# soedinglab/MMseqs2

Hardware: AMD Instinct MI355X
Metric: sw_gcells_per_s (higher is better)
Workload: dtype int16

## Files before the change

### mmseqs2_amd/csrc/pf_kernels.hip

```cpp
#include <type_traits>

#include "mmgpu_internal.h"
#include "pf_device.h"

namespace mmgpu {

namespace {

__device__ __forceinline__ PfCand *cand_slot(const PfDedupArgs &A, uint64_t bucket, uint32_t k) {
    return k < (uint32_t)PF_CAND0 ? A.cand_small + bucket * PF_CAND0 + k : A.cand + (A.cand_base[bucket] - A.cand_origin) + k;
}

struct __attribute__((packed, aligned(4))) U32Pair {
    uint32_t a, b;
};
struct __attribute__((packed, aligned(4))) U32Quad {
    uint32_t a, b, c, d;
};


constexpr uint32_t PF_COFS_KMERS = 12, PF_COFS_DWORDS = 4;

__global__ __launch_bounds__(256) void pf_cofs_kernel(const uint32_t *offsets, uint64_t table, uint32_t *cofs) {
    const uint64_t blk = (uint64_t)blockIdx.x * 256u + threadIdx.x;
// ... 447 lines not shown
            if (chunk_end > cur) cur = chunk_end;
            L += 64;
            r = rn;
            if (L >= Lend) break;
        }
    }
    __syncthreads();

    const int nbits = pf_bin_shift(B);
    constexpr int ROUNDS = PF_T / (64 * SPW);
    uint64_t ent[ROUNDS];
    uint32_t rk[ROUNDS];
    uint16_t *mycnt = cnt + (uint32_t)wave * B;
#pragma unroll
    for (int r = 0; r < ROUNDS; r++) {
        const uint32_t slot = (uint32_t)wave * (PF_T / SPW) + (uint32_t)r * 64u + (uint32_t)lane;
        const bool valid = slot < tile_n;
        ent[r] = valid ? stage[slot] : 0ull;
        const uint32_t bin = (uint32_t)ent[r] & (B - 1);
        const uint64_t m = match_lanes(bin, nbits, valid);
        const uint32_t rank = (uint32_t)__popcll(m & lanes_below(lane));
        uint32_t c = 0;
        if (valid) c = mycnt[bin];
        rk[r] = c + rank;
        if (valid && rank == 0) mycnt[bin] = (uint16_t)(c + (uint32_t)__popcll(m));
    }
    __syncthreads();

    {
        const uint32_t bpt = B >= 256 ? B / 256 : 1;
        const uint32_t b0 = threadIdx.x * bpt;
        uint32_t s = 0;
        if (b0 < B)
            for (uint32_t b = b0; b < b0 + bpt; b++)
                for (int w = 0; w < SPW; w++) s += cnt[(uint32_t)w * B + b];
        const uint32_t incl = wave_incl_scan(s);
        if (lane == 63) wsum[wave] = incl;
        __syncthreads();
        uint32_t run = incl - s;
        for (int w = 0; w < wave; w++) run += wsum[w];
        if (b0 < B) {
            uint16_t *bo = A.bin_off + (size_t)t * (B + 1);
            for (uint32_t b = b0; b < b0 + bpt; b++) {
                bo[b] = (uint16_t)run;
                uint32_t tot = 0;
                for (int w = 0; w < SPW; w++) {
                    const uint32_t c = cnt[(uint32_t)w * B + b];
                    cnt[(uint32_t)w * B + b] = (uint16_t)(run + tot);
                    tot += c;
                }
                if (tot) atomicAdd(&A.bucket_count[(size_t)q * B + b], tot);
                run += tot;
            }
            if (b0 + bpt == B) bo[B] = (uint16_t)run;
        }
    }
    __syncthreads();

    uint32_t *stage_w = reinterpret_cast<uint32_t *>(stage);
    uint8_t *stage_h = reinterpret_cast<uint8_t *>(stage) + (size_t)PF_T * 4;
#pragma unroll
    for (int r = 0; r < ROUNDS; r++) {
        const uint32_t slot = (uint32_t)wave * (PF_T / SPW) + (uint32_t)r * 64u + (uint32_t)lane;
        if (slot < tile_n) {
            const uint32_t id = (uint32_t)ent[r];
            const uint32_t bin = id & (B - 1);
            const uint32_t diag = (uint32_t)(ent[r] >> 32) & 0xFFFFu;
            const uint32_t at = mycnt[bin] + rk[r];
            stage_w[at] = (id >> nbits) | ((diag & 0xFFu) << 12) | ((uint32_t)(ent[r] >> 48) << 20);
            stage_h[at] = (uint8_t)(diag >> 8);
        }
    }
    __syncthreads();
    uint32_t *dst = A.split + (size_t)t * PF_T;
    uint32_t *dst_h = reinterpret_cast<uint32_t *>(A.split_hi + (size_t)t * PF_T);
    const uint32_t *src_h = reinterpret_cast<const uint32_t *>(stage_h);
    for (uint32_t s = threadIdx.x; s < tile_n; s += (uint32_t)SPW * 64u) dst[s] = stage_w[s];
    for (uint32_t s = threadIdx.x; s < (tile_n + 3u) / 4u; s += (uint32_t)SPW * 64u) dst_h[s] = src_h[s];
}

struct Seg {
    int a, b, P, M;
};
__device__ __forceinline__ Seg seg_combine(const Seg &l, const Seg &r) {
    Seg o;
    o.b = l.b + r.b;
    o.a = max(r.a, l.a + r.b);
    o.P = max(l.P, l.b + r.P);
    o.M = max(max(l.M, r.M), l.a + r.P);
    return o;
}
template <int NW>
__device__ __forceinline__ void load_cells(const uint8_t *p, uint32_t (&w)[NW]) {
    static_assert(NW == 4 || NW == 6, "16 or 24 bytes");
    const uintptr_t u = reinterpret_cast<uintptr_t>(p);
    const uint32_t *a = reinterpret_cast<const uint32_t *>(u & ~(uintptr_t)3);
    const uint32_t sh = (uint32_t)(u & 3u);
    const U32Quad d = *reinterpret_cast<const U32Quad *>(a);
    w[0] = __builtin_amdgcn_alignbyte(d.b, d.a, sh);
    w[1] = __builtin_amdgcn_alignbyte(d.c, d.b, sh);
    w[2] = __builtin_amdgcn_alignbyte(d.d, d.c, sh);
    if constexpr (NW == 4) {
        w[3] = __builtin_amdgcn_alignbyte(a[4], d.d, sh);
    } else {
        typedef uint32_t u32x3 __attribute__((ext_vector_type(3)));
        const u32x3 e = *reinterpret_cast<const u32x3 *>(a + 4);
        w[3] = __builtin_amdgcn_alignbyte(e.x, d.d, sh);
        w[4] = __builtin_amdgcn_alignbyte(e.y, e.x, sh);
        w[5] = __builtin_amdgcn_alignbyte(e.z, e.y, sh);
    }
}
template <int NW>
__device__ __forceinline__ Seg seg_cells_n(const uint32_t (&tw)[NW], const uint32_t (&qw)[NW], const uint32_t (&cw)[NW], int nn,
                                           const int8_t *smat) {
    Seg g;
    g.a = 0; g.b = 0; g.P = -(1 << 28); g.M = 0;
#pragma unroll
    for (int k = 0; k < 4 * NW; k++) {
        const uint32_t t5 = (tw[k >> 2] >> ((k & 3) * 8)) & 31u;
        const uint32_t q5 = (qw[k >> 2] >> ((k & 3) * 8)) & 31u;
        const int cb = (int)(int8_t)((cw[k >> 2] >> ((k & 3) * 8)) & 0xFFu);
        int x = (int)(int8_t)(smat[(q5 << 5) | t5] + cb);
        x = k < nn ? x : 0;
        g.b += x;
        g.a = max(0, g.a + x);
        g.P = max(g.P, g.b);
        g.M = max(g.M, g.a);
    }
    return g;
}
template <int NW>
__device__ __forceinline__ Seg seg_cells_rows_n(const uint32_t (&tw)[NW], const int8_t *rows, int nn) {
    Seg g;
    g.a = 0; g.b = 0; g.P = -(1 << 28); g.M = 0;
#pragma unroll
    for (int k = 0; k < 4 * NW; k++) {
        if (k < nn) {
            const int tb_ = (int)((tw[k >> 2] >> ((k & 3) * 8)) & 0xFFu);
            const int x = (int)rows[k * PF_PROW + (tb_ & (PF_PROW - 1))];
            g.b += x;
            g.a = max(0, g.a + x);
            g.P = max(g.P, g.b);
            g.M = max(g.M, g.a);
        }
    }
    return g;
}
__device__ __forceinline__ Seg seg_tree16(Seg g, int gl) {
#pragma unroll
    for (int d = 1; d < 16; d <<= 1) {
        Seg r;
        r.a = __shfl_down(g.a, d);
        r.b = __shfl_down(g.b, d);
        r.P = __shfl_down(g.P, d);
        r.M = __shfl_down(g.M, d);
        if ((gl & (2 * d - 1)) == 0) g = seg_combine(g, r);
    }
    return g;
}

template <bool SLOTS = true>
__device__ __forceinline__ uint64_t score_chunk(const PfDedupArgs &A, const int8_t *smat, uint64_t bucket, uint32_t q, uint32_t cb0,
                                                uint32_t nin, uint32_t ncand, PfCand c, int bshift, uint32_t *score_out = nullptr) {
    const int lane = lane_id();
    const int grp = lane >> 4, gl = lane & 15;
    const uint32_t qp0 = A.q_off[q];
    const int qlen = (int)(A.q_off[q + 1] - qp0);
    const uint8_t *qr = A.q_res + qp0;
    const uint8_t *qc = reinterpret_cast<const uint8_t *>(A.q_corr) + qp0;
    const bool has = (uint32_t)lane < nin;
    const int8_t *prows = (A.q_isprof && A.q_isprof[q]) ? A.q_rows + (size_t)qp0 * PF_PROW : nullptr;
    int my_len = 0, my_qs = 0;
    unsigned long long my_addr = 0;
    uint64_t cells = 0;
    if (has && !(A.q_nseg && A.q_nseg[q]))
        c.diag = (uint16_t)((c.diag & 0xFFu) | ((uint32_t)A.split_hi[(size_t)A.q_tile_base[q] * PF_T + c.score] << 8));
    if (has) {
        const int d = (int)(short)c.diag;
        const int tlen = (int)A.t_len[c.id];
        const uint8_t *t = A.t_res + (size_t)A.t_off4[c.id] * 4;
        const int mind = d < 0 ? -d : d;
        int ts = 0;
        if (d >= 0 && mind < qlen) {
            my_len = min(tlen, qlen - mind);
            my_qs = mind;
        } else if (d < 0 && mind < tlen) {
            my_len = min(tlen - mind, qlen);
            ts = mind;
        }
        my_addr = (unsigned long long)reinterpret_cast<uintptr_t>(t + ts);
        cells = (uint64_t)my_len;
        if (tlen >= 32768 && A.q_flags) atomicOr(&A.q_flags[q], 1u);
    }
    int my_score = 0;
    constexpr int UN = 2;
    auto trip = [&](auto nw_tag, const uint32_t k0) {
        constexpr int NW = decltype(nw_tag)::value;
        constexpr int CPL = 4 * NW, PASS = 16 * CPL;
        uint32_t tw[UN][NW], qw[UN][NW], cw[UN][NW];
        int len_u[UN], qs_u[UN];
        unsigned long long addr_u[UN];
#pragma unroll
        for (int u = 0; u < UN; u++) {
            const int src = (int)k0 + u * 4 + grp;
            len_u[u] = __shfl(my_len, src);
            qs_u[u] = __shfl(my_qs, src);
            addr_u[u] = __shfl(my_addr, src);
            if ((uint32_t)src >= nin) len_u[u] = 0;
#pragma unroll
            for (int z = 0; z < NW; z++) { tw[u][z] = 0; qw[u][z] = 0; cw[u][z] = 0; }
            if (gl * CPL < len_u[u]) {
                load_cells<NW>(reinterpret_cast<const uint8_t *>((uintptr_t)addr_u[u]) + gl * CPL, tw[u]);
                if (!prows) {
                    load_cells<NW>(qr + qs_u[u] + gl * CPL, qw[u]);
                    load_cells<NW>(qc + qs_u[u] + gl * CPL, cw[u]);
                }
            }
        }
#pragma unroll
        for (int u = 0; u < UN; u++) {
            const int len = len_u[u];
            Seg g;
            g.a = 0; g.b = 0; g.P = -(1 << 28); g.M = 0;
            if (gl * CPL < len) {
                if (prows) g = seg_cells_rows_n<NW>(tw[u], prows + (size_t)(qs_u[u] + gl * CPL) * PF_PROW, min(CPL, len - gl * CPL));
                else g = seg_cells_n<NW>(tw[u], qw[u], cw[u], min(CPL, len - gl * CPL), smat);
            }
            g = seg_tree16(g, gl);
            int sc = 0, best = 0;
            if (gl == 0 && len > 0) {
                best = max(g.M, g.P);
                sc = max(g.a, g.b);
            }
            int maxlen = len;
            maxlen = max(maxlen, __shfl_xor(maxlen, 16));
            maxlen = max(maxlen, __shfl_xor(maxlen, 32));
            for (int p0 = PASS; p0 < maxlen; p0 += PASS) {
                const int o = p0 + gl * CPL;
                Seg h;
                h.a = 0; h.b = 0; h.P = -(1 << 28); h.M = 0;
                if (o < len) {
                    uint32_t t2[NW], q2[NW], c2[NW];
                    load_cells<NW>(reinterpret_cast<const uint8_t *>((uintptr_t)addr_u[u]) + o, t2);
                    if (prows) h = seg_cells_rows_n<NW>(t2, prows + (size_t)(qs_u[u] + o) * PF_PROW, min(CPL, len - o));
                    else {
                        load_cells<NW>(qr + qs_u[u] + o, q2);
                        load_cells<NW>(qc + qs_u[u] + o, c2);
                        h = seg_cells_n<NW>(t2, q2, c2, min(CPL, len - o), smat);
                    }
                }
                h = seg_tree16(h, gl);
                if (gl == 0 && p0 < len) {
                    best = max(best, max(h.M, sc + h.P));
                    sc = max(h.a, sc + h.b);
                }
            }
            const int r0 = __shfl(best, 0), r1 = __shfl(best, 16), r2 = __shfl(best, 32), r3 = __shfl(best, 48);
            const int rel = lane - ((int)k0 + u * 4);
            if (rel >= 0 && rel < 4) my_score = rel == 0 ? r0 : (rel == 1 ? r1 : (rel == 2 ? r2 : r3));
        }
    };
    for (uint32_t k0 = 0; k0 < nin; k0 += 4 * UN) {
        const bool mine = (uint32_t)lane >= k0 && (uint32_t)lane < k0 + 4u * UN && has;
        if (ballot(mine && my_len > 256)) trip(std::integral_constant<int, 6>{}, k0);
        else trip(std::integral_constant<int, 4>{}, k0);
    }
    c.score = (uint32_t)my_score;
    if (score_out) *score_out = c.score;
    if constexpr (!SLOTS) return cells;
    if (has) {
        PfCand *slot = cand_slot(A, bucket, cb0 + (uint32_t)lane);
        slot->score = c.score;
        slot->diag = c.diag;
    }
    if (ncand <= 64 && !A.nucl) {
        const uint32_t cnt = min(255u, c.score);
        const uint64_t same = match_lanes(c.id >> bshift, 12, has);
        bool win = has;
        uint64_t m = same & ~(1ull << lane);
        while (ballot(m != 0)) {
            const int o = m ? __ffsll((long long)m) - 1 : lane;
            const uint32_t oc = __shfl(cnt, o);
            if (m) {
                if (oc > cnt || (oc == cnt && o < lane)) win = false;
                m &= m - 1;
            }
        }
        win = win && cnt >= A.min_diag_score;
        const uint64_t wb = ballot(win);
        if (wb) {
            PfCand *surv = A.surv + (A.cand_base[(uint64_t)q * A.bins] - A.cand_origin);
            uint32_t base = 0;
            if (lane == 0) base = atomicAdd(&A.surv_count[q], (uint32_t)__popcll(wb));
            base = __shfl(base, 0);
            if (win) surv[base + (uint32_t)__popcll(wb & lanes_below(lane))] = c;
        }
    }
    return cells;
}

constexpr int REPLAY_WAVES_PER_EU = 4;
constexpr int REPLAY_PD = 4;


struct ReplayLds {
    uint32_t prev[4][PF_IDS_PER_BIN / 4];
    uint32_t last[4][PF_IDS_PER_BIN / 4];
    uint32_t emit[4][PF_IDS_PER_BIN / 32];
    uint32_t cand[4][3][64];
    uint8_t mark[4][64];
    int8_t smat[32 * 32];
};

__device__ __forceinline__ uint32_t lds_byte_exchange(uint32_t *word, uint32_t shift, uint32_t byte) {
    uint32_t old;
    const uint32_t addr = (uint32_t)(uintptr_t)word;
    asm volatile("ds_mskor_rtn_b32 %0, %1, %2, %3\n\ts_waitcnt lgkmcnt(0)" : "=v"(old) : "v"(addr), "v"(0xFFu << shift), "v"(byte << shift) : "memory");
    return old;
}

template <bool SEGS>
__device__ __forceinline__ void replay_bucket_impl(const PfDedupArgs &A, ReplayLds &M, uint64_t bucket) {
    const int lane = lane_id(), wave = (int)(threadIdx.x >> 6);
    const uint32_t B = A.bins;
    const uint32_t q = (uint32_t)(bucket / B), bin = (uint32_t)(bucket % B);
    const uint32_t ntiles = A.q_ntiles[q];
    if (ntiles == 0) {
        if (lane == 0) A.cand_count[bucket] = 0;
        return;
    }
    const uint32_t tb = A.q_tile_base[q];
    uint32_t *P = M.prev[wave];
    uint32_t *L = M.last[wave];
    uint32_t *E = M.emit[wave];
    uint8_t *mark = M.mark[wave];
    const int bshift = pf_bin_shift(B);
    auto clear_state = [&]() {
        uint4 *P4 = reinterpret_cast<uint4 *>(P);
        for (int k = lane; k < PF_IDS_PER_BIN / 16; k += 64) P4[k] = make_uint4(0u, 0u, 0u, 0u);
        for (int k = lane; k < PF_IDS_PER_BIN / 32; k += 64) E[k] = 0;
    };
    clear_state();

    uint32_t ncand = 0;
    const uint64_t below = lanes_below(lane);
    PfCand *const cand_small = A.cand_small + bucket * PF_CAND0;
    PfCand *const cand_big = A.cand + (A.cand_base[bucket] - A.cand_origin);
    const uint8_t *const split_hi_q = A.split_hi + (size_t)tb * PF_T;
    const uint32_t *const split_q = A.split + (size_t)tb * PF_T;
    const uint32_t nseg = SEGS ? A.q_nseg[q] : 0u;
// ... 24 lines not shown
            const uint32_t d_m = (uint32_t)__shfl((int)seg_delta, m);
            tile_out = t0 + (uint32_t)m;
            at_out = (uint32_t)(x + d_m);
            e_out = split_q[x < total ? (size_t)tile_out * PF_T + at_out : (size_t)0];
        };
        auto one_round = [&](const uint32_t x0, uint32_t &e_slot, uint32_t &tile_slot, uint32_t &at_slot) {
            const uint32_t e = e_slot;
            const uint32_t tile_cur = tile_slot;
            const uint32_t where = tile_cur * (uint32_t)PF_T + at_slot;
            const bool act = x0 + (uint32_t)lane < total;
            request(x0 + 64u * REPLAY_PD, e_slot, tile_slot, at_slot);
            const uint32_t key = e & 0xFFFu;
            const uint32_t d8 = (e >> 12) & 0xFFu;
            const uint32_t arr = tile_cur * (uint32_t)PF_T + (e >> 20);
            const uint32_t sh = (key & 3u) * 8u;
            uint64_t todo = SEGS ? ballot(act) : 1ull;
            while (todo) {
                const bool now = SEGS ? (act && ((todo >> lane) & 1ull) && arr < next_boundary) : act;
                if (!SEGS || ballot(now)) {
                    bool flag = false;
                    if (now) flag = ((lds_byte_exchange(&P[key >> 2], sh, d8) >> sh) & 0xFFu) == d8;
                    if (ballot(flag)) {
                        bool keep = false;
                        if (flag) {
                            const uint32_t bit = 1u << (key & 31u);
                            const bool emitted_before = (atomicOr(&E[key >> 5], bit) & bit) != 0u;
                            const uint32_t last_byte = (lds_byte_exchange(&L[key >> 2], sh, d8) >> sh) & 0xFFu;
                            keep = !emitted_before || last_byte != d8;
                        }
                        const uint64_t kb = ballot(keep);
                        if (keep) {
                            PfCand c;
                            c.id = (key << bshift) | bin;
                            c.arr = arr;
                            c.score = SEGS ? 0u : where;
                            c.diag = (uint16_t)(SEGS ? (d8 | ((uint32_t)split_hi_q[where] << 8)) : d8);
                            c.pad = (uint16_t)cur_seg;
                            const uint32_t ck = ncand + (uint32_t)__popcll(kb & below);
                            *(ck < (uint32_t)PF_CAND0 ? cand_small + ck : cand_big + ck) = c;
                            if (!SEGS && ck < 64) {
                                M.cand[wave][0][ck] = key | (d8 << 12);
                                M.cand[wave][1][ck] = arr;
                                M.cand[wave][2][ck] = where;
                            }
                        }
                        ncand += (uint32_t)__popcll(kb);
                    }
                }
                if (!SEGS) break;
                todo &= ~ballot(now);
                if (todo) {
                    clear_state();
                    cur_seg++;
                    next_boundary = cur_seg + 1 <= nseg ? segs[cur_seg + 1] : 0xFFFFFFFFu;
                }
            }
        };
        static_assert(REPLAY_PD == 4, "four named slots below");
        uint32_t e0, e1, e2, e3, tile0, tile1, tile2, tile3, at0, at1, at2, at3;
        request(0u, e0, tile0, at0);
        request(64u, e1, tile1, at1);
        request(128u, e2, tile2, at2);
        request(192u, e3, tile3, at3);
        for (uint32_t xg = 0; xg < total; xg += 64u * REPLAY_PD) {
            one_round(xg, e0, tile0, at0);
            one_round(xg + 64u, e1, tile1, at1);
            one_round(xg + 128u, e2, tile2, at2);
            one_round(xg + 192u, e3, tile3, at3);
        }
    }
    if (lane == 0) {
        A.cand_count[bucket] = ncand;
        if (!SEGS && ncand > 64 && A.big_list) A.big_list[atomicAdd(A.big_count, 1u)] = (uint32_t)(bucket - (uint64_t)A.q_first * B);
    }
    if (!SEGS && ncand > 0 && ncand <= 64) {
        PfCand c = pf_cand_zero();
        if ((uint32_t)lane < ncand) {
            const uint32_t kd = M.cand[wave][0][lane];
            c.id = ((kd & 0xFFFu) << bshift) | bin;
            c.arr = M.cand[wave][1][lane];
            c.diag = (uint16_t)(kd >> 12);
            c.score = M.cand[wave][2][lane];
        }
        uint64_t cells = score_chunk(A, M.smat, bucket, q, 0, ncand, ncand, c, bshift);
        if (A.cell_counter) wave_sum_to((unsigned long long *)&A.cell_counter[q], cells);
    }
}

__global__ __launch_bounds__(256) __attribute__((amdgpu_waves_per_eu(REPLAY_WAVES_PER_EU))) void pf_replay_kernel(PfDedupArgs A) {
    __shared__ ReplayLds M;
    pf_load_smat32<256>(M.smat, A.mat, A.alphabet);
    __syncthreads();
    uint64_t bucket;
    if (!pf_wave_bucket(A, 4u, &bucket)) return;
    if (A.q_nseg && A.q_nseg[(uint32_t)(bucket / A.bins)]) replay_bucket_impl<true>(A, M, bucket);
    else replay_bucket_impl<false>(A, M, bucket);
}

__device__ __forceinline__ void ungapped_bucket(const PfDedupArgs &A, const int8_t *smat, uint64_t bucket) {
    const int lane = lane_id();
    const uint32_t B = A.bins;
    const uint32_t ncand = A.cand_count[bucket];
    const uint32_t q = (uint32_t)(bucket / B);
    if (ncand <= 64 || (A.q_nseg && A.q_nseg[q])) return;
    const int bshift = pf_bin_shift(B);
    uint64_t cells = 0;
    for (uint32_t cb0 = 0; cb0 < ncand; cb0 += 64) {
        const uint32_t nin = min(64u, ncand - cb0);
        PfCand c = pf_cand_zero();
        if ((uint32_t)lane < nin) c = *cand_slot(A, bucket, cb0 + (uint32_t)lane);
        cells += score_chunk(A, smat, bucket, q, cb0, nin, ncand, c, bshift);
    }
    if (A.cell_counter) wave_sum_to((unsigned long long *)&A.cell_counter[q], cells);
}

__global__ __launch_bounds__(256) void pf_ungapped_kernel(PfDedupArgs A) {
    __shared__ int8_t smat[32 * 32];
    const int wave = (int)(threadIdx.x >> 6);
    pf_load_smat32<256>(smat, A.mat, A.alphabet);
    __syncthreads();
    const uint32_t B = A.bins;
    if (A.big_list) {
        const uint32_t n = *A.big_count;
        for (uint32_t i = blockIdx.x * 4u + (uint32_t)wave; i < n; i += gridDim.x * 4u) ungapped_bucket(A, smat, (uint64_t)A.q_first * B + A.big_list[i]);
        return;
    }
    const uint64_t bucket = (uint64_t)A.q_first * B + (uint64_t)blockIdx.x * 4u + (uint32_t)wave;
    if (bucket >= (uint64_t)(A.q_first + A.n_queries) * B) return;
    ungapped_bucket(A, smat, bucket);
}

__global__ __launch_bounds__(256) void pf_count_kernel(PfDedupArgs A) {
    __shared__ uint16_t s_state[4][PF_IDS_PER_BIN];
    __shared__ uint32_t s_emit[4][PF_IDS_PER_BIN / 32];
    const int lane = lane_id(), wave = (int)(threadIdx.x >> 6);
    const uint32_t B = A.bins;
    uint64_t bucket;
    if (!pf_wave_bucket(A, 4u, &bucket)) return;
    const uint32_t q = (uint32_t)(bucket / B), bin = (uint32_t)(bucket % B);
    const uint32_t ntiles = A.q_ntiles[q];
    if (lane == 0) A.cand_count[bucket] = 0;
    if (ntiles == 0) return;
    const uint32_t tb = A.q_tile_base[q];
    uint16_t *S = s_state[wave];
    uint32_t *E = s_emit[wave];
    const int bshift = pf_bin_shift(B);
    for (int k = lane; k < PF_IDS_PER_BIN; k += 64) S[k] = 0;
    for (int k = lane; k < PF_IDS_PER_BIN / 32; k += 64) E[k] = 0;
    uint32_t ncand = 0;
    const uint64_t below = lanes_below(lane);
    for (uint32_t t0 = 0; t0 < ntiles; t0 += 64) {
        const uint32_t tl = t0 + (uint32_t)lane;
        uint32_t o0 = 0, n = 0;
        if (tl < ntiles) {
            const uint16_t *bo = A.bin_off + (size_t)(tb + tl) * (B + 1) + bin;
            o0 = bo[0];
            n = (uint32_t)bo[1] - o0;
        }
        const uint32_t incl = wave_incl_scan(n);
        const uint32_t total = __shfl(incl, 63);
        const uint32_t excl = incl - n;
        for (uint32_t x0 = 0; x0 < total; x0 += 64) {
            const uint32_t x = x0 + (uint32_t)lane;
            const bool now = x < total;
            const int m = seg_find(excl, now ? x : 0u);
            const uint32_t ex_m = __shfl(excl, m), o_m = __shfl(o0, m);
            const uint32_t tile = t0 + (uint32_t)m;
            uint32_t e = 0;
            const size_t where = (size_t)(tb + tile) * PF_T + o_m + (x - ex_m);
            if (now) e = A.split[where];
            const uint32_t key = e & 0xFFFu;
            const uint32_t id = (key << bshift) | bin;
            const uint32_t d8 = (e >> 12) & 0xFFu;
            const uint32_t arr = tile * (uint32_t)PF_T + (e >> 20);
            const uint64_t same = match_lanes(key, 12, now);
            uint32_t st = 0, em = 0;
            if (now) {
                st = S[key];
                em = (E[key >> 5] >> (key & 31u)) & 1u;
            }
            const uint64_t pm = same & below;
            const int pl = pm ? highest_lane(pm) : lane;
            const uint32_t d_pl = __shfl(d8, pl);
            const uint32_t prevd = pm ? d_pl : (st & 0xFFu);
            const bool flag = now && d8 == prevd;
            const uint64_t fl = ballot(flag);
            const uint64_t fm = same & fl;
            if (now && (same & ~below & ~(1ull << lane)) == 0) {
                const uint32_t cnt = min(255u, (st >> 8) + (uint32_t)__popcll(fm));
                S[key] = (uint16_t)(d8 | (cnt << 8));
            }
            const bool keep = flag && (fm & below) == 0 && em == 0u;
            if (keep) atomicOr(&E[key >> 5], 1u << (key & 31u));
            const uint64_t kb = ballot(keep);
            if (keep) {
                PfCand c;
                c.id = id;
                c.arr = arr;
                c.score = 0;
                c.diag = (uint16_t)(d8 | ((uint32_t)A.split_hi[where] << 8));
                c.pad = 0;
                *cand_slot(A, bucket, ncand + (uint32_t)__popcll(kb & below)) = c;
            }
            ncand += (uint32_t)__popcll(kb);
        }
    }
    if (ncand == 0) return;
    __threadfence();
    if (lane == 0 && A.q_ncand) {
        const uint32_t before = atomicAdd(&A.q_ncand[q], ncand);
        if (before + ncand >= A.sort_cap && A.q_flags) atomicOr(&A.q_flags[q], 2u);
    }
// ... 38 lines not shown
            c = *cand_slot(A, bucket, ci);
            const uint32_t cnt = min(255u, c.score);
            win = S[c.id >> bshift] == keepmax_key(cnt, ci) && cnt >= A.min_diag_score;
        }
        wave_append(&A.surv_count[q], surv, win, c);
    }
}

__global__ __launch_bounds__(256) void pf_keepmax_kernel(PfDedupArgs A) {
    __shared__ uint32_t s_tab[4][PF_IDS_PER_BIN];
    const int wave = (int)(threadIdx.x >> 6);
    if (A.nucl) return;
    uint64_t bucket;
    if (!pf_wave_bucket(A, 4u, &bucket)) return;
    keepmax_bucket(A, s_tab[wave], bucket);
}

__global__ __launch_bounds__(1024) void pf_keepmax_list_kernel(PfDedupArgs A) {
    __shared__ uint32_t S[PF_IDS_PER_BIN];
    const uint32_t B = A.bins;
    const int bshift = pf_bin_shift(B);
    const uint32_t n = *A.big_count;
    for (uint32_t i = blockIdx.x; i < n; i += gridDim.x) {
        const uint64_t bucket = (uint64_t)A.q_first * B + A.big_list[i];
        const uint32_t ncand = A.cand_count[bucket];
        const uint32_t q = (uint32_t)(bucket / B);
        for (uint32_t k = threadIdx.x; k < (uint32_t)PF_IDS_PER_BIN; k += 1024) S[k] = 0;
        __syncthreads();
        for (uint32_t ci = threadIdx.x; ci < ncand; ci += 1024) {
            const PfCand *cp = cand_slot(A, bucket, ci);
            atomicMax(&S[cp->id >> bshift], keepmax_key(min(255u, cp->score), ci));
        }
        __syncthreads();
        PfCand *surv = A.surv + (A.cand_base[(uint64_t)q * B] - A.cand_origin);
        for (uint32_t c0 = 0; c0 < ncand; c0 += 1024) {
            const uint32_t ci = c0 + threadIdx.x;
            bool win = false;
            PfCand c = pf_cand_zero();
            if (ci < ncand) {
                c = *cand_slot(A, bucket, ci);
                const uint32_t cnt = min(255u, c.score);
                win = S[c.id >> bshift] == keepmax_key(cnt, ci) && cnt >= A.min_diag_score;
            }
            wave_append(&A.surv_count[q], surv, win, c);
        }
        __syncthreads();
    }
}

constexpr int PF_LONG_POOL = 4096;
constexpr uint32_t PF_LONG_NONE = 0xFFFFu;

__device__ int wave_diag_score(const int8_t *smat, const uint8_t *qr, const uint8_t *qc, const int8_t *prows, int qlen, const uint8_t *t,
                               int tlen, int diag) {
    const int lane = lane_id();
    const int mind = diag < 0 ? -diag : diag;
    int len, qs, ts;
    if (diag >= 0 && mind < qlen) {
        len = min(tlen, qlen - mind);
        qs = mind;
        ts = 0;
    } else if (diag < 0 && mind < tlen) {
        len = min(tlen - mind, qlen);
        qs = 0;
        ts = mind;
    } else {
        return 0;
    }
    int sc = 0, best = 0;
    for (int p0 = 0; p0 < len; p0 += 1024) {
        const int o = p0 + lane * 16;
        Seg h;
        h.a = 0; h.b = 0; h.P = -(1 << 28); h.M = 0;
        if (o < len) {
            uint32_t tw[4], qw[4], cw[4];
            load_cells<4>(t + ts + o, tw);
            if (prows) h = seg_cells_rows_n<4>(tw, prows + (size_t)(qs + o) * PF_PROW, min(16, len - o));
            else {
                load_cells<4>(qr + qs + o, qw);
                load_cells<4>(qc + qs + o, cw);
                h = seg_cells_n<4>(tw, qw, cw, min(16, len - o), smat);
            }
        }
        h = seg_tree16(h, lane & 15);
        Seg g[4];
#pragma unroll
        for (int k = 0; k < 4; k++) {
            g[k].a = __shfl(h.a, 16 * k);
            g[k].b = __shfl(h.b, 16 * k);
            g[k].P = __shfl(h.P, 16 * k);
            g[k].M = __shfl(h.M, 16 * k);
        }
        const Seg all = seg_combine(seg_combine(g[0], g[1]), seg_combine(g[2], g[3]));
        best = max(best, max(all.M, sc + all.P));
        sc = max(all.a, sc + all.b);
    }
    return best;
}

__device__ int wave_long_score(const int8_t *smat, const uint8_t *qr, const uint8_t *qc, const int8_t *prows, int qlen, const uint8_t *t,
                               int tlen, uint32_t diag16) {
    int total = 0;
    for (uint32_t d = 1; d <= 1u + (uint32_t)tlen / 32768u; d++)
        total = max(total, wave_diag_score(smat, qr, qc, prows, qlen, t, tlen, (int)(0u - d * 65536u + diag16)));
    for (uint32_t d = 0; d <= (uint32_t)qlen / 65536u; d++)
        total = max(total, wave_diag_score(smat, qr, qc, prows, qlen, t, tlen, (int)(d * 65536u + diag16)));
    return total;
}

__global__ __launch_bounds__(256) void pf_longq_kernel(PfDedupArgs A) {
    __shared__ int8_t smat[32 * 32];
    const int lane = lane_id();
    pf_load_smat32<256>(smat, A.mat, A.alphabet);
    __syncthreads();
    const uint32_t B = A.bins;
    uint64_t bucket;
    if (!pf_wave_bucket(A, 4u, &bucket)) return;
    const uint32_t q = (uint32_t)(bucket / B);
    const uint32_t qp0 = A.q_off[q];
    const int qlen = (int)(A.q_off[q + 1] - qp0);
    if (qlen < 32768) return;
    if (lane == 0 && bucket == (uint64_t)q * B) atomicOr(&A.q_flags[q], 1u);
    if (A.nucl || (A.q_nseg && A.q_nseg[q])) return;
    const uint8_t *qr = A.q_res + qp0;
    const uint8_t *qc = reinterpret_cast<const uint8_t *>(A.q_corr) + qp0;
    const int8_t *prows = (A.q_isprof && A.q_isprof[q]) ? A.q_rows + (size_t)qp0 * PF_PROW : nullptr;
    const uint32_t ncand = A.cand_count[bucket];
    for (uint32_t ci = 0; ci < ncand; ci++) {
        PfCand *slot = cand_slot(A, bucket, ci);
        const uint32_t id = slot->id;
        const int own = wave_long_score(smat, qr, qc, prows, qlen, A.t_res + (size_t)A.t_off4[id] * 4, (int)A.t_len[id], slot->diag);
        if (lane == 0) slot->score = (uint32_t)own;
    }
}

__global__ __launch_bounds__(256) void pf_long_kernel(PfDedupArgs A) {
    __shared__ uint32_t s_tab[PF_IDS_PER_BIN];
    __shared__ uint32_t s_dbits[65536 / 32];
    __shared__ uint64_t s_key[PF_LONG_POOL];
    __shared__ uint32_t s_ci[PF_LONG_POOL];
    __shared__ uint16_t s_bucket[PF_LONG_POOL];
    __shared__ uint16_t s_job[PF_LONG_POOL];
    __shared__ int8_t smat[32 * 32];
    __shared__ uint32_t sh_npool, sh_nlong;
    const uint32_t q = A.q_first + blockIdx.x;
    if (!(A.q_flags[q] & 1u)) return;
    if (A.nucl || (A.q_nseg && A.q_nseg[q])) return;
    const int lane = lane_id(), wave = (int)(threadIdx.x >> 6);
    const uint32_t B = A.bins;
    const int bshift = pf_bin_shift(B);
    pf_load_smat32<256>(smat, A.mat, A.alphabet);
    for (int k = (int)threadIdx.x; k < 65536 / 32; k += 256) s_dbits[k] = 0;
    if (threadIdx.x == 0) {
        sh_npool = 0;
        sh_nlong = 0;
    }
    __syncthreads();
    const uint32_t qp0 = A.q_off[q];
    const int qlen = (int)(A.q_off[q + 1] - qp0);
    if (qlen < 32768) {
    for (uint32_t bk = (uint32_t)wave; bk < B; bk += 4) {
        const uint64_t bucket = (uint64_t)q * B + bk;
        const uint32_t ncand = A.cand_count[bucket];
        for (uint32_t ci = (uint32_t)lane; ci < ncand; ci += 64) {
            const PfCand *cp = cand_slot(A, bucket, ci);
            if (A.t_len[cp->id] >= 32768u) atomicOr(&s_dbits[cp->diag >> 5], 1u << (cp->diag & 31u));
        }
    }
    __syncthreads();
    const uint32_t refmask = A.ref_bins - 1;
    for (uint32_t bk = (uint32_t)wave; bk < B; bk += 4) {
        const uint64_t bucket = (uint64_t)q * B + bk;
        const uint32_t ncand = A.cand_count[bucket];
        for (uint32_t ci = (uint32_t)lane; ci < ncand; ci += 64) {
            const PfCand *cp = cand_slot(A, bucket, ci);
            const uint32_t d = cp->diag;
// ... 265 lines not shown
        for (uint32_t r0 = 0; r0 < n; r0 += 64) {
            const bool act = r0 + (uint32_t)lane < n;
            const uint32_t idx = act ? n - 1u - (r0 + (uint32_t)lane) : 0u;
            PfOvfElem e;
            e.id = 0; e.score = 0; e.ord = 0; e.diag = 0; e.pad0 = 0; e.pad1 = 0;
            if (act) e = O[idx];
            const uint32_t d8 = e.diag & 0xFFu, key = e.id >> bshift;
            const uint64_t same = match_lanes(key, 12, act);
            const uint64_t pm = same & below;
            const int pl = pm ? highest_lane(pm) : lane;
            const uint32_t d_pl = __shfl(d8, pl);
            uint32_t prev = 0;
            if (act) prev = pm ? d_pl : tab[key];
            const bool keep = act && (e.score != 0 || prev != d8);
            if (act && (same & ~below & ~(1ull << lane)) == 0) tab[key] = d8;
            const uint64_t kb = ballot(keep);
            if (keep) {
                e.ord = -e.ord;
                S[m + (uint32_t)__popcll(kb & below)] = e;
            }
            m += (uint32_t)__popcll(kb);
        }
        n = m;
        cur = S;
    } else if (do_merge && final_step) {
        for (uint32_t r0 = 0; r0 < n; r0 += 64) {
            const bool act = r0 + (uint32_t)lane < n;
            const uint32_t idx = act ? n - 1u - (r0 + (uint32_t)lane) : 0u;
            uint32_t id = 0, d8 = 0;
            if (act) { id = O[idx].id; d8 = O[idx].diag & 0xFFu; }
            const uint32_t key = id >> bshift;
            const uint64_t same = match_lanes(key, 12, act);
            if (act && (same & ~below & ~(1ull << lane)) == 0) tab[key] = (d8 + 1u) & 0xFFu;
        }
        uint32_t m = 0;
        for (uint32_t r0 = 0; r0 < n; r0 += 64) {
            const uint32_t idx = r0 + (uint32_t)lane;
            const bool act = idx < n;
            PfOvfElem e;
            e.id = 0; e.score = 0; e.ord = 0; e.diag = 0; e.pad0 = 0; e.pad1 = 0;
            if (act) e = O[idx];
            const uint32_t d8 = e.diag & 0xFFu, key = e.id >> bshift;
            const uint64_t same = match_lanes(key, 12, act);
            const uint64_t pm = same & below;
            const int pl = pm ? highest_lane(pm) : lane;
            const uint32_t d_pl = __shfl(d8, pl);
            uint32_t prev = 0;
            if (act) prev = pm ? d_pl : tab[key];
            const bool keep = act && prev != d8;
            if (act && (same & ~below & ~(1ull << lane)) == 0) tab[key] = d8;
            const uint64_t kb = ballot(keep);
            if (keep) S[m + (uint32_t)__popcll(kb & below)] = e;
            m += (uint32_t)__popcll(kb);
        }
        n = m;
        cur = S;
    }
    __threadfence();
    const bool do_score = final_step || (step > 1 && prev_total != 0);
    if (!do_score) {
        if (lane == 0) {
            A.o_count[(size_t)qi * B + bin] = n;
            if (n) atomicAdd(&totals[step], n);
        }
        return;
    }
    for (uint32_t r0 = 0; r0 < n; r0 += 64) {
        const uint32_t idx = r0 + (uint32_t)lane;
        const bool need = idx < n && cur[idx].score == 0;
        const uint64_t nb = ballot(need);
        if (!nb) continue;
        const uint32_t cnt = (uint32_t)__popcll(nb), mine = (uint32_t)__popcll(nb & below);
        if (need) tab[mine] = (uint32_t)lane;
        __builtin_amdgcn_wave_barrier();
        const int src = (uint32_t)lane < cnt ? (int)tab[lane] : 0;
        const uint32_t my_id = idx < n ? cur[idx].id : 0u, my_diag = idx < n ? (uint32_t)cur[idx].diag : 0u;
        PfCand c;
        c.id = (uint32_t)__shfl((int)my_id, src);
        c.arr = 0;
        c.score = 0;
        c.diag = (uint16_t)__shfl((int)my_diag, src);
        c.pad = 0;
        uint32_t sc = 0;
        (void)score_chunk<false>(D, smat, bucket, q, 0, cnt, 65u, c, bshift, &sc);
        tab[64 + lane] = sc;
        __builtin_amdgcn_wave_barrier();
        if (need) cur[idx].score = tab[64 + mine];
    }
    __threadfence();
    for (int k = lane; k < PF_IDS_PER_BIN; k += 64) tab[k] = 0;
    for (uint32_t r0 = 0; r0 < n; r0 += 64) {
        const uint32_t idx = r0 + (uint32_t)lane;
        if (idx < n) {
            const uint32_t cnt = min(255u, cur[idx].score);
            atomicMax(&tab[cur[idx].id >> bshift], keepmax_key(cnt, idx));
        }
    }
    PfOvfElem *dst = cur == O ? S : O;
    uint32_t m = 0;
    PfCand *surv = D.surv + (D.cand_base[(uint64_t)q * B] - D.cand_origin);
    for (uint32_t r0 = 0; r0 < n; r0 += 64) {
        const uint32_t idx = r0 + (uint32_t)lane;
        bool keep = false;
        PfOvfElem e;
        e.id = 0; e.score = 0; e.ord = 0; e.diag = 0; e.pad0 = 0; e.pad1 = 0;
        if (idx < n) {
            e = cur[idx];
            const uint32_t cnt = min(255u, e.score);
            const uint32_t first = 0xFFFFFFu - (tab[e.id >> bshift] & 0xFFFFFFu);
            keep = idx == first || (cnt == 0 && idx > first);
            if (final_step) keep = keep && cnt >= D.min_diag_score;
        }
        const uint64_t kb = ballot(keep);
        if (final_step) {
            if (kb) {
                uint32_t sb = 0;
                if (lane == 0) sb = atomicAdd(&D.surv_count[q], (uint32_t)__popcll(kb));
                sb = __shfl(sb, 0);
                if (keep) {
                    const unsigned long long o45 = (unsigned long long)(e.ord + (1ll << 40));
                    PfCand c;
                    c.id = e.id;
                    c.arr = (uint32_t)o45;
                    c.score = e.score;
                    c.diag = e.diag;
                    c.pad = (uint16_t)(o45 >> 32);
                    surv[sb + (uint32_t)__popcll(kb & below)] = c;
                }
            }
        } else if (keep) {
            dst[m + (uint32_t)__popcll(kb & below)] = e;
        }
        m += (uint32_t)__popcll(kb);
    }
    if (!final_step) {
        __threadfence();
        if (dst != O) {
            for (uint32_t r0 = 0; r0 < m; r0 += 64) {
                const uint32_t idx = r0 + (uint32_t)lane;
                if (idx < m) O[idx] = dst[idx];
            }
        }
        if (lane == 0) {
            A.o_count[(size_t)qi * B + bin] = m;
            if (m) atomicAdd(&totals[step], m);
        }
    }
}

__device__ uint32_t list_ordinal(const PfSelectArgs &A, uint32_t q, uint32_t arr) {
    const uint32_t p0 = A.q_off[q], p1 = A.q_off[q + 1];
    uint32_t lo = p0, hi = p1 - 1;
    while (lo < hi) {
        const uint32_t mid = (lo + hi + 1) >> 1;
        if (A.peb[mid] <= arr) lo = mid; else hi = mid - 1;
    }
    const uint32_t rel = arr - A.peb[lo];
    uint32_t a = A.list_base[lo], b = A.list_base[lo + 1];
    if (b <= a) return a - A.list_base[p0];
    b -= 1;
    while (a < b) {
        const uint32_t mid = (a + b + 1) >> 1;
        if (A.lists[mid].lprefix <= rel) a = mid; else b = mid - 1;
    }
    return a - A.list_base[p0];
}

// ... 389 lines not shown
```

Baseline: 4502.

## Pack candidate diagonals into 16-cell units and score with a DPP segmented wave scan

Replaces the per-group scoring of ungapped diagonals (four candidates per 16-lane group, tree reductions, extra passes for long diagonals) with a load-balanced scheme. Every candidate's diagonal is split into 16-cell units, units from all candidates are packed contiguously across the 64 lanes, and a segmented max-plus scan built on DPP row moves combines them, carrying state across passes. The aim is to remove idle lanes on short or uneven diagonals and to replace shuffle-based reductions with cheaper DPP moves. In exchange it adds a shared-memory mark array and per-pass scans to map lanes to owners, drops the 24-byte load path, and changes the long-diagonal reduction to use the same scan.

New measurement: 4492. Within noise of the previous version (-0.2%).

```diff
diff --git a/mmseqs2_amd/csrc/pf_kernels.hip b/mmseqs2_amd/csrc/pf_kernels.hip
--- a/mmseqs2_amd/csrc/pf_kernels.hip
+++ b/mmseqs2_amd/csrc/pf_kernels.hip
@@ -553,6 +553,11 @@
 struct Seg {
     int a, b, P, M;
 };
+__device__ __forceinline__ Seg seg_identity() {
+    Seg g;
+    g.a = 0; g.b = 0; g.P = -(1 << 28); g.M = 0;
+    return g;
+}
 __device__ __forceinline__ Seg seg_combine(const Seg &l, const Seg &r) {
     Seg o;
     o.b = l.b + r.b;
@@ -561,31 +566,26 @@
     o.M = max(max(l.M, r.M), l.a + r.P);
     return o;
 }
+typedef uint32_t U32x4 __attribute__((ext_vector_type(4), aligned(4)));
 template <int NW>
 __device__ __forceinline__ void load_cells(const uint8_t *p, uint32_t (&w)[NW]) {
-    static_assert(NW == 4 || NW == 6, "16 or 24 bytes");
+    static_assert(NW == 4, "16 bytes");
+    typedef const __attribute__((address_space(1))) uint32_t *GlobalWords;
+    typedef const __attribute__((address_space(1))) U32x4 *GlobalQuad;
     const uintptr_t u = reinterpret_cast<uintptr_t>(p);
-    const uint32_t *a = reinterpret_cast<const uint32_t *>(u & ~(uintptr_t)3);
+    const uintptr_t a = u & ~(uintptr_t)3;
     const uint32_t sh = (uint32_t)(u & 3u);
-    const U32Quad d = *reinterpret_cast<const U32Quad *>(a);
-    w[0] = __builtin_amdgcn_alignbyte(d.b, d.a, sh);
-    w[1] = __builtin_amdgcn_alignbyte(d.c, d.b, sh);
-    w[2] = __builtin_amdgcn_alignbyte(d.d, d.c, sh);
-    if constexpr (NW == 4) {
-        w[3] = __builtin_amdgcn_alignbyte(a[4], d.d, sh);
-    } else {
-        typedef uint32_t u32x3 __attribute__((ext_vector_type(3)));
-        const u32x3 e = *reinterpret_cast<const u32x3 *>(a + 4);
-        w[3] = __builtin_amdgcn_alignbyte(e.x, d.d, sh);
-        w[4] = __builtin_amdgcn_alignbyte(e.y, e.x, sh);
-        w[5] = __builtin_amdgcn_alignbyte(e.z, e.y, sh);
-    }
+    const U32x4 d = *(GlobalQuad)a;
+    const uint32_t e = ((GlobalWords)a)[4];
+    w[0] = __builtin_amdgcn_alignbyte(d.y, d.x, sh);
+    w[1] = __builtin_amdgcn_alignbyte(d.z, d.y, sh);
+    w[2] = __builtin_amdgcn_alignbyte(d.w, d.z, sh);
+    w[3] = __builtin_amdgcn_alignbyte(e, d.w, sh);
 }
 template <int NW>
 __device__ __forceinline__ Seg seg_cells_n(const uint32_t (&tw)[NW], const uint32_t (&qw)[NW], const uint32_t (&cw)[NW], int nn,
                                            const int8_t *smat) {
-    Seg g;
-    g.a = 0; g.b = 0; g.P = -(1 << 28); g.M = 0;
+    Seg g = seg_identity();
 #pragma unroll
     for (int k = 0; k < 4 * NW; k++) {
         const uint32_t t5 = (tw[k >> 2] >> ((k & 3) * 8)) & 31u;
@@ -602,8 +602,7 @@
 }
 template <int NW>
 __device__ __forceinline__ Seg seg_cells_rows_n(const uint32_t (&tw)[NW], const int8_t *rows, int nn) {
-    Seg g;
-    g.a = 0; g.b = 0; g.P = -(1 << 28); g.M = 0;
+    Seg g = seg_identity();
 #pragma unroll
     for (int k = 0; k < 4 * NW; k++) {
         if (k < nn) {
@@ -617,24 +616,41 @@
     }
     return g;
 }
-__device__ __forceinline__ Seg seg_tree16(Seg g, int gl) {
-#pragma unroll
-    for (int d = 1; d < 16; d <<= 1) {
-        Seg r;
-        r.a = __shfl_down(g.a, d);
-        r.b = __shfl_down(g.b, d);
-        r.P = __shfl_down(g.P, d);
-        r.M = __shfl_down(g.M, d);
-        if ((gl & (2 * d - 1)) == 0) g = seg_combine(g, r);
-    }
+template <int CTRL, int ROW_MASK, bool BOUND>
+__device__ __forceinline__ Seg seg_move(const Seg &g) {
+    Seg r;
+    r.a = __builtin_amdgcn_update_dpp(0, g.a, CTRL, ROW_MASK, 0xF, BOUND);
+    r.b = __builtin_amdgcn_update_dpp(0, g.b, CTRL, ROW_MASK, 0xF, BOUND);
+    r.P = __builtin_amdgcn_update_dpp(0, g.P, CTRL, ROW_MASK, 0xF, BOUND);
+    r.M = __builtin_amdgcn_update_dpp(0, g.M, CTRL, ROW_MASK, 0xF, BOUND);
+    return r;
+}
+__device__ __forceinline__ Seg seg_take(bool ok, const Seg &l, const Seg &g) {
+    const Seg c = seg_combine(l, g);
+    Seg o;
+    o.a = ok ? c.a : g.a;
+    o.b = ok ? c.b : g.b;
+    o.P = ok ? c.P : g.P;
+    o.M = ok ? c.M : g.M;
+    return o;
+}
+__device__ __forceinline__ Seg seg_scan64(Seg g, int lane, int head) {
+    const int row = lane & ~15;
+    const int lo = max(head, row);
+    g = seg_take(lane - 1 >= lo, seg_move<0x111 , 0xF, true>(g), g);
+    g = seg_take(lane - 2 >= lo, seg_move<0x112 , 0xF, true>(g), g);
+    g = seg_take(lane - 4 >= lo, seg_move<0x114 , 0xF, true>(g), g);
+    g = seg_take(lane - 8 >= lo, seg_move<0x118 , 0xF, true>(g), g);
+    g = seg_take((lane & 16) != 0 && head < row, seg_move<0x142 , 0xA, false>(g), g);
+    g = seg_take(lane >= 32 && head < 32, seg_move<0x143 , 0xC, false>(g), g);
     return g;
 }
 
 template <bool SLOTS = true>
 __device__ __forceinline__ uint64_t score_chunk(const PfDedupArgs &A, const int8_t *smat, uint64_t bucket, uint32_t q, uint32_t cb0,
-                                                uint32_t nin, uint32_t ncand, PfCand c, int bshift, uint32_t *score_out = nullptr) {
+                                                uint32_t nin, uint32_t ncand, PfCand c, int bshift, uint8_t *mark,
+                                                uint32_t *score_out = nullptr) {
     const int lane = lane_id();
-    const int grp = lane >> 4, gl = lane & 15;
     const uint32_t qp0 = A.q_off[q];
     const int qlen = (int)(A.q_off[q + 1] - qp0);
     const uint8_t *qr = A.q_res + qp0;
@@ -663,80 +679,71 @@
         cells = (uint64_t)my_len;
         if (tlen >= 32768 && A.q_flags) atomicOr(&A.q_flags[q], 1u);
     }
-    int my_score = 0;
-    constexpr int UN = 2;
-    auto trip = [&](auto nw_tag, const uint32_t k0) {
-        constexpr int NW = decltype(nw_tag)::value;
-        constexpr int CPL = 4 * NW, PASS = 16 * CPL;
-        uint32_t tw[UN][NW], qw[UN][NW], cw[UN][NW];
-        int len_u[UN], qs_u[UN];
-        unsigned long long addr_u[UN];
-#pragma unroll
-        for (int u = 0; u < UN; u++) {
-            const int src = (int)k0 + u * 4 + grp;
-            len_u[u] = __shfl(my_len, src);
-            qs_u[u] = __shfl(my_qs, src);
-            addr_u[u] = __shfl(my_addr, src);
-            if ((uint32_t)src >= nin) len_u[u] = 0;
-#pragma unroll
-            for (int z = 0; z < NW; z++) { tw[u][z] = 0; qw[u][z] = 0; cw[u][z] = 0; }
-            if (gl * CPL < len_u[u]) {
-                load_cells<NW>(reinterpret_cast<const uint8_t *>((uintptr_t)addr_u[u]) + gl * CPL, tw[u]);
-                if (!prows) {
-                    load_cells<NW>(qr + qs_u[u] + gl * CPL, qw[u]);
-                    load_cells<NW>(qc + qs_u[u] + gl * CPL, cw[u]);
-                }
-            }
-        }
-#pragma unroll
-        for (int u = 0; u < UN; u++) {
-            const int len = len_u[u];
+    const uint32_t units = ((uint32_t)my_len + 15u) >> 4;
+    const uint32_t incl = wave_incl_scan(units);
+    const uint32_t base = incl - units;
+    const uint32_t U = (uint32_t)__builtin_amdgcn_readlane((int)incl, 63);
+    int sc = 0, best = 0;
+    auto deal = [&](auto prof_tag) {
+        constexpr bool PROF = decltype(prof_tag)::value;
+        const int first = __ffsll((long long)ballot(units != 0u)) - 1;
+        const unsigned long long addr0 = __shfl(my_addr, first);
+        const uint8_t *const idle_t = reinterpret_cast<const uint8_t *>(
+            (uintptr_t)(((unsigned long long)(uint32_t)__builtin_amdgcn_readfirstlane((int)(addr0 >> 32)) << 32) |
+                        (uint32_t)__builtin_amdgcn_readfirstlane((int)(uint32_t)addr0)));
+        const int idle_q = __builtin_amdgcn_readlane(my_qs, first);
+        int m_carry = 0;
+        for (uint32_t x0 = 0; x0 < U; x0 += 64u) {
+            mark[lane] = 0;
+            const uint32_t rel = base - x0;
+            if (units != 0u && rel < 64u) mark[rel] = (uint8_t)lane;
+            asm volatile("" ::: "memory");
+            int m = (int)mark[lane];
+            m = max(wave_incl_max_scan(m), m_carry);
+            m_carry = __builtin_amdgcn_readlane(m, 63);
+            const int len_o = __shfl(my_len, m);
+            const int qs_o = __shfl(my_qs, m);
+            const unsigned long long addr_o = __shfl(my_addr, m);
+            const uint32_t base_o = (uint32_t)__shfl((int)base, m);
+            const uint32_t x = x0 + (uint32_t)lane;
+            const bool act = x < U;
+            const int off = (int)((x - base_o) << 4);
+            const int nn = act ? min(16, len_o - off) : 0;
+            const int head = max((int)(base_o - x0), 0);
+            const uint8_t *tp = act ? reinterpret_cast<const uint8_t *>((uintptr_t)addr_o) + off : idle_t;
+            const int qo = act ? qs_o + off : idle_q;
+            uint32_t tw[4];
+            load_cells<4>(tp, tw);
             Seg g;
-            g.a = 0; g.b = 0; g.P = -(1 << 28); g.M = 0;
-            if (gl * CPL < len) {
-                if (prows) g = seg_cells_rows_n<NW>(tw[u], prows + (size_t)(qs_u[u] + gl * CPL) * PF_PROW, min(CPL, len - gl * CPL));
-                else g = seg_cells_n<NW>(tw[u], qw[u], cw[u], min(CPL, len - gl * CPL), smat);
-            }
-            g = seg_tree16(g, gl);
-            int sc = 0, best = 0;
-            if (gl == 0 && len > 0) {
-                best = max(g.M, g.P);
-                sc = max(g.a, g.b);
-            }
-            int maxlen = len;
-            maxlen = max(maxlen, __shfl_xor(maxlen, 16));
-            maxlen = max(maxlen, __shfl_xor(maxlen, 32));
-            for (int p0 = PASS; p0 < maxlen; p0 += PASS) {
-                const int o = p0 + gl * CPL;
-                Seg h;
-                h.a = 0; h.b = 0; h.P = -(1 << 28); h.M = 0;
-                if (o < len) {
-                    uint32_t t2[NW], q2[NW], c2[NW];
-                    load_cells<NW>(reinterpret_cast<const uint8_t *>((uintptr_t)addr_u[u]) + o, t2);
-                    if (prows) h = seg_cells_rows_n<NW>(t2, prows + (size_t)(qs_u[u] + o) * PF_PROW, min(CPL, len - o));
-                    else {
-                        load_cells<NW>(qr + qs_u[u] + o, q2);
-                        load_cells<NW>(qc + qs_u[u] + o, c2);
-                        h = seg_cells_n<NW>(t2, q2, c2, min(CPL, len - o), smat);
-                    }
-                }
-                h = seg_tree16(h, gl);
-                if (gl == 0 && p0 < len) {
-                    best = max(best, max(h.M, sc + h.P));
-                    sc = max(h.a, sc + h.b);
-                }
-            }
-            const int r0 = __shfl(best, 0), r1 = __shfl(best, 16), r2 = __shfl(best, 32), r3 = __shfl(best, 48);
-            const int rel = lane - ((int)k0 + u * 4);
-            if (rel >= 0 && rel < 4) my_score = rel == 0 ? r0 : (rel == 1 ? r1 : (rel == 2 ? r2 : r3));
+            if constexpr (PROF) {
+                g = seg_cells_rows_n<4>(tw, prows + (size_t)qo * PF_PROW, nn);
+            } else {
+                uint32_t qw[4], cw[4];
+                load_cells<4>(qr + qo, qw);
+                load_cells<4>(qc + qo, cw);
+                g = seg_cells_n<4>(tw, qw, cw, nn, smat);
+                g.P = nn > 0 ? g.P : -(1 << 28);
+            }
+            g = seg_scan64(g, lane, head);
+            const uint32_t end = base + units;
+            const bool meets = units != 0u && base < x0 + 64u && end > x0;
+            const int src = (int)((min(end, x0 + 64u) - x0 - 1u) & 63u);
+            Seg h;
+            h.a = __shfl(g.a, src);
+            h.b = __shfl(g.b, src);
+            h.P = __shfl(g.P, src);
+            h.M = __shfl(g.M, src);
+            if (meets) {
+                best = max(best, max(h.M, sc + h.P));
+                sc = max(h.a, sc + h.b);
+            }
         }
     };
-    for (uint32_t k0 = 0; k0 < nin; k0 += 4 * UN) {
-        const bool mine = (uint32_t)lane >= k0 && (uint32_t)lane < k0 + 4u * UN && has;
-        if (ballot(mine && my_len > 256)) trip(std::integral_constant<int, 6>{}, k0);
-        else trip(std::integral_constant<int, 4>{}, k0);
-    }
-    c.score = (uint32_t)my_score;
+    if (U != 0u) {
+        if (prows) deal(std::true_type{});
+        else deal(std::false_type{});
+    }
+    c.score = (uint32_t)best;
     if (score_out) *score_out = c.score;
     if constexpr (!SLOTS) return cells;
     if (has) {
@@ -927,7 +934,7 @@
             c.diag = (uint16_t)(kd >> 12);
             c.score = M.cand[wave][2][lane];
         }
-        uint64_t cells = score_chunk(A, M.smat, bucket, q, 0, ncand, ncand, c, bshift);
+        uint64_t cells = score_chunk(A, M.smat, bucket, q, 0, ncand, ncand, c, bshift, mark);
         if (A.cell_counter) wave_sum_to((unsigned long long *)&A.cell_counter[q], cells);
     }
 }
@@ -942,7 +949,7 @@
     else replay_bucket_impl<false>(A, M, bucket);
 }
 
-__device__ __forceinline__ void ungapped_bucket(const PfDedupArgs &A, const int8_t *smat, uint64_t bucket) {
+__device__ __forceinline__ void ungapped_bucket(const PfDedupArgs &A, const int8_t *smat, uint8_t *mark, uint64_t bucket) {
     const int lane = lane_id();
     const uint32_t B = A.bins;
     const uint32_t ncand = A.cand_count[bucket];
@@ -954,25 +961,26 @@
         const uint32_t nin = min(64u, ncand - cb0);
         PfCand c = pf_cand_zero();
         if ((uint32_t)lane < nin) c = *cand_slot(A, bucket, cb0 + (uint32_t)lane);
-        cells += score_chunk(A, smat, bucket, q, cb0, nin, ncand, c, bshift);
+        cells += score_chunk(A, smat, bucket, q, cb0, nin, ncand, c, bshift, mark);
     }
     if (A.cell_counter) wave_sum_to((unsigned long long *)&A.cell_counter[q], cells);
 }
 
 __global__ __launch_bounds__(256) void pf_ungapped_kernel(PfDedupArgs A) {
     __shared__ int8_t smat[32 * 32];
+    __shared__ uint8_t mark[4][64];
     const int wave = (int)(threadIdx.x >> 6);
     pf_load_smat32<256>(smat, A.mat, A.alphabet);
     __syncthreads();
     const uint32_t B = A.bins;
     if (A.big_list) {
         const uint32_t n = *A.big_count;
-        for (uint32_t i = blockIdx.x * 4u + (uint32_t)wave; i < n; i += gridDim.x * 4u) ungapped_bucket(A, smat, (uint64_t)A.q_first * B + A.big_list[i]);
+        for (uint32_t i = blockIdx.x * 4u + (uint32_t)wave; i < n; i += gridDim.x * 4u) ungapped_bucket(A, smat, mark[wave], (uint64_t)A.q_first * B + A.big_list[i]);
         return;
     }
     const uint64_t bucket = (uint64_t)A.q_first * B + (uint64_t)blockIdx.x * 4u + (uint32_t)wave;
     if (bucket >= (uint64_t)(A.q_first + A.n_queries) * B) return;
-    ungapped_bucket(A, smat, bucket);
+    ungapped_bucket(A, smat, mark[wave], bucket);
 }
 
 __global__ __launch_bounds__(256) void pf_count_kernel(PfDedupArgs A) {
@@ -1177,16 +1185,12 @@
                 h = seg_cells_n<4>(tw, qw, cw, min(16, len - o), smat);
             }
         }
-        h = seg_tree16(h, lane & 15);
-        Seg g[4];
-#pragma unroll
-        for (int k = 0; k < 4; k++) {
-            g[k].a = __shfl(h.a, 16 * k);
-            g[k].b = __shfl(h.b, 16 * k);
-            g[k].P = __shfl(h.P, 16 * k);
-            g[k].M = __shfl(h.M, 16 * k);
-        }
-        const Seg all = seg_combine(seg_combine(g[0], g[1]), seg_combine(g[2], g[3]));
+        h = seg_scan64(h, lane, 0);
+        Seg all;
+        all.a = __builtin_amdgcn_readlane(h.a, 63);
+        all.b = __builtin_amdgcn_readlane(h.b, 63);
+        all.P = __builtin_amdgcn_readlane(h.P, 63);
+        all.M = __builtin_amdgcn_readlane(h.M, 63);
         best = max(best, max(all.M, sc + all.P));
         sc = max(all.a, sc + all.b);
     }
@@ -1618,7 +1622,7 @@
         c.diag = (uint16_t)__shfl((int)my_diag, src);
         c.pad = 0;
         uint32_t sc = 0;
-        (void)score_chunk<false>(D, smat, bucket, q, 0, cnt, 65u, c, bshift, &sc);
+        (void)score_chunk<false>(D, smat, bucket, q, 0, cnt, 65u, c, bshift, reinterpret_cast<uint8_t *>(tab + 128), &sc);
         tab[64 + lane] = sc;
         __builtin_amdgcn_wave_barrier();
         if (need) cur[idx].score = tab[64 + mine];
```
